# zhvng/open-musiclm

Measured on NVIDIA H100. Metric: coarse-stage training tokens/sec (positions fed to the transformer per optimiser step / step time), higher is better.
Workload: dtype bf16 (fp16 operands for the forward GEMMs on LayerNorm outputs x weights; fp32 accumulate)

## Files before the change

### open-musiclm_b200/csrc/attn_bwd_tc.cu

```cuda
#include "common.cuh"
#include "ptx.cuh"
#include "../../include/omlm_b200.h"
#include <stdlib.h>
#include <algorithm>
#include <array>
#include <functional>
#include <map>
#include <mutex>
#include <vector>

namespace omlm {

constexpr int kBtThreads = 384;
constexpr int kBtBQ = 64, kBtBK = 128;
constexpr float kBtL2e = 1.4426950408889634f;

constexpr int kBoK = 0, kBoV = 16384, kBoQ = 32768 , kBoDO = 49152 ;
constexpr int kBoP = 65536 , kBoDS = 81920 , kBoBar = 98304 ;
constexpr int kBoSds = 98368;
constexpr int kBtMaxSmem = 232448;
constexpr int kBtSdsLd = 72;
constexpr int kBoWin = kBoSds + 2 * 64 * kBtSdsLd * 4;

static int bt_win_ld(int h) { return ((62 + h) / h + 64 + 23) / 32 * 32 + 8; }

__device__ __forceinline__ float bt_ex2(float x) {
  float y;
  asm("ex2.approx.ftz.f32 %0, %1;" : "=f"(y) : "f"(x));
  return y;
}
__device__ __forceinline__ void bt_red2(float* addr, float a, float b) {
  asm volatile("red.global.add.v2.f32 [%0], {%1, %2};" ::"l"(addr), "f"(a), "f"(b) : "memory");
}
__device__ __forceinline__ void bt_cp_async4(float* dst, const float* src) {
  asm volatile("cp.async.ca.shared.global [%0], [%1], 4;" ::"r"(smem_u32(dst)), "l"(src) : "memory");
}

__device__ __forceinline__ int bt_ld_acquire(const int* p) {
  int v;
  asm volatile("ld.acquire.gpu.global.b32 %0, [%1];" : "=r"(v) : "l"(p) : "memory");
  return v;
}
__device__ __forceinline__ unsigned long long bt_globaltimer() {
  unsigned long long t;
  asm volatile("mov.u64 %0, %%globaltimer;" : "=l"(t));
  return t;
}
__device__ __noinline__ void bt_wait_turn(const int* ctr, int turn, int* err) {
  const unsigned long long t0 = bt_globaltimer();
  while (bt_ld_acquire(ctr) != turn) {
    if (*reinterpret_cast<volatile int*>(err) != 0) return;
    if (bt_globaltimer() - t0 > 4000000000ull) { atomicExch(err, 1); return; }
    __nanosleep(64);
  }
}
__device__ __forceinline__ void bt_pass_turn(int* ctr) {
  asm volatile("red.release.gpu.global.add.s32 [%0], 1;" ::"l"(ctr) : "memory");
}

struct BtDet {
  int* turn_dq;
  int* turn_kv;
  int* meta;
  int* err;
  float* dpart;
};

template <bool DET>
__global__ void __launch_bounds__(kBtThreads, 1)
attn_bwd_tc_kernel(const __grid_constant__ CUtensorMap tmQ, const __grid_constant__ CUtensorMap tmDO,
                   const __grid_constant__ CUtensorMap tmKV, const float* __restrict__ lse2, const float* __restrict__ dsum,
                   const float* __restrict__ table, int table_ld, const unsigned char* __restrict__ key_mask,
                   float* __restrict__ dqn, float* __restrict__ dkvn, float* __restrict__ dtable, int N, int h, float scale,
                   int Wacc, int win_ld, int tiles_per_chunk, int nbatch, const BtDet det) {
  extern __shared__ __align__(1024) uint8_t smem_raw[];
  uint8_t* smem = smem_raw + ((1024u - (smem_u32(smem_raw) & 1023u)) & 1023u);
  uint64_t* bars = reinterpret_cast<uint64_t*>(smem + kBoBar);
  uint64_t* kv_full = bars + 0;
  uint64_t* qd_full = bars + 1;
  uint64_t* qd_empty = bars + 3;
  float* dacc = reinterpret_cast<float*>(smem + kBoWin) + 2 * h * win_ld;

  const int wg = threadIdx.x >> 7, lane = threadIdx.x & 31;
  const int R = N * h;
  const int n_rt = (R + kBtBQ - 1) / kBtBQ;
  const int n_kt = (N + kBtBK - 1) / kBtBK;
  const int b = blockIdx.x % nbatch;
  int u = blockIdx.x / nbatch, kt = 0;
  for (; kt < n_kt; ++kt) {
    const int cnt = (n_rt - (kt * kBtBK * h) / kBtBQ + tiles_per_chunk - 1) / tiles_per_chunk;
    if (u < cnt) break;
    u -= cnt;
  }
  const int j0 = kt * kBtBK;
  const int rt0 = (j0 * h) / kBtBQ + u * tiles_per_chunk;
  const int rt1 = min(n_rt, rt0 + tiles_per_chunk);
  const int T = rt1 - rt0;
  const int i_lo = (rt0 * kBtBQ) / h, i_hi = min(N - 1, (rt1 * kBtBQ - 1) / h);
  const int dmin = max(0, i_lo - j0 - (kBtBK - 1));
  const int wacc_used = i_hi - j0 - dmin + 1;

  if (threadIdx.x == 0) {
    tma_prefetch_desc(&tmQ); tma_prefetch_desc(&tmDO); tma_prefetch_desc(&tmKV);
    mbar_init(kv_full, 1);
    for (int i = 0; i < 2; ++i) { mbar_init(&qd_full[i], 1); mbar_init(&qd_empty[i], 2); }
    fence_barrier_init();
  }
  for (int x = threadIdx.x; x < 2 * h * Wacc; x += blockDim.x) dacc[x] = 0.f;
  __syncthreads();

  if (wg == 0) {
    asm volatile("setmaxnreg.dec.sync.aligned.u32 40;");
    if (threadIdx.x == 0) {
      mbar_expect_tx(kv_full, 2 * 16384);
      tma_load_2d(smem + kBoK, &tmKV, kv_full, 0, b * N + j0);
      tma_load_2d(smem + kBoV, &tmKV, kv_full, 64, b * N + j0);
      for (int t = 0; t < T; ++t) {
        const int st = t & 1;
        mbar_wait(&qd_empty[st], ((t >> 1) & 1) ^ 1);
        mbar_expect_tx(&qd_full[st], 2 * 8192);
        tma_load_2d(smem + kBoQ + st * 8192, &tmQ, &qd_full[st], 0, b * R + (rt0 + t) * kBtBQ);
        tma_load_2d(smem + kBoDO + st * 8192, &tmDO, &qd_full[st], 0, b * R + (rt0 + t) * kBtBQ);
      }
    }
  } else {
    asm volatile("setmaxnreg.inc.sync.aligned.u32 232;");
    const int cw = wg - 1;
    const int wq = (threadIdx.x >> 5) & 3, qr = lane >> 2, qc = lane & 3;
    const bool leader = (threadIdx.x & 127) == 0;
    const int kbase = j0 + cw * 64;
    const uint32_t sk = smem_u32(smem + kBoK) + cw * 8192, sv = smem_u32(smem + kBoV) + cw * 8192;
    uint8_t* p_tile = smem + kBoP + cw * 8192;
    uint8_t* ds_tile = smem + kBoDS + cw * 8192;
    float* sdsf = reinterpret_cast<float*>(smem + kBoSds) + cw * 64 * kBtSdsLd;
    float* win = reinterpret_cast<float*>(smem + kBoWin) + cw * h * win_ld;
    float* wacc = dacc + cw * h * Wacc;
    const int tid128 = threadIdx.x & 127;
    const uint32_t sp = smem_u32(p_tile), sds = smem_u32(ds_tile);
    const float sc2 = scale * kBtL2e;
    uint32_t vis = 0;
#pragma unroll
    for (int c = 0; c < 8; ++c)
#pragma unroll
      for (int e = 0; e < 2; ++e) {
        const int j = kbase + 8 * c + 2 * qc + e;
        if (j < N && (key_mask == nullptr || key_mask[static_cast<long long>(b) * N + j] != 0)) vis |= 1u << (2 * c + e);
      }
    auto fetch_tile = [&](int rb, float (&lse)[2], float (&D)[2]) {
      const int it_lo = min(rb, R - 1) / h, it_hi = min(rb + kBtBQ - 1, R - 1) / h;
      const int win_w = it_hi - it_lo + 64, dlo = it_lo - kbase - 63;
      for (int hh = tid128 / win_w, w = tid128 - hh * win_w; hh < h;) {
        if (dlo + w >= 0) bt_cp_async4(win + hh * win_ld + w, table + hh * static_cast<long>(table_ld) + dlo + w);
        for (w += 128; w >= win_w; ++hh) w -= win_w;
      }
      asm volatile("cp.async.commit_group;" ::: "memory");
#pragma unroll
      for (int hr = 0; hr < 2; ++hr) {
        const int rc = min(rb + wq * 16 + qr + hr * 8, R - 1);
        lse[hr] = lse2[static_cast<long long>(b) * R + rc];
        D[hr] = dsum[static_cast<long long>(b) * R + rc];
      }
    };
    float lse_t[2], D_t[2];
    fetch_tile(rt0 * kBtBQ, lse_t, D_t);
    float dv[32], dk[32];
#pragma unroll
    for (int x = 0; x < 32; ++x) { dv[x] = 0.f; dk[x] = 0.f; }
    mbar_wait(kv_full, 0);
    for (int t = 0; t < T; ++t) {
      const int st = t & 1;
      const int rbase = (rt0 + t) * kBtBQ;
      const uint32_t sq = smem_u32(smem + kBoQ + st * 8192), sdo = smem_u32(smem + kBoDO + st * 8192);
      mbar_wait(&qd_full[st], (t >> 1) & 1);
      float s[32], dp[32];
      wgmma_fence();
#pragma unroll
      for (int ks = 0; ks < 4; ++ks) {
        Wgmma<64, false>::ss<0, 0>(s, make_smem_desc(sq + ks * 32, 16, 1024), make_smem_desc(sk + ks * 32, 16, 1024), ks > 0 ? 1u : 0u);
        Wgmma<64, false>::ss<0, 0>(dp, make_smem_desc(sdo + ks * 32, 16, 1024), make_smem_desc(sv + ks * 32, 16, 1024), ks > 0 ? 1u : 0u);
      }
      wgmma_commit();
      const int it_lo = min(rbase, R - 1) / h, it_hi = min(rbase + kBtBQ - 1, R - 1) / h;
      asm volatile("cp.async.wait_all;" ::: "memory");
      asm volatile("bar.sync %0, 128;" ::"r"(1 + cw) : "memory");
      wgmma_wait<0>();
      wgmma_reg_fence(s);
      wgmma_reg_fence(dp);
#pragma unroll
      for (int hr = 0; hr < 2; ++hr) {
        const int lr = wq * 16 + qr + hr * 8;
        const int r = rbase + lr;
        const bool row_ok = r < R;
        const int rc = min(r, R - 1);
        const int i = rc / h, hh = rc - i * h;
        const float lse = lse_t[hr], D = D_t[hr];
        const float* wrow = win + hh * win_ld + i - it_lo + 63 - 2 * qc;
        const int dcol = i - kbase - 2 * qc;
        uint8_t* prow = p_tile + lr * 128;
        uint8_t* drow = ds_tile + lr * 128;
        float wv[16];
#pragma unroll
        for (int x = 0; x < 16; ++x) wv[x] = wrow[-8 * (x >> 1) - (x & 1)];
#pragma unroll
        for (int c = 0; c < 8; ++c) {
          float pp[2], dd[2];
#pragma unroll
          for (int e = 0; e < 2; ++e) {
            const bool live = row_ok && ((vis >> (2 * c + e)) & 1u) && dcol >= 8 * c + e;
            const float x = s[4 * c + 2 * hr + e];
            pp[e] = live ? bt_ex2(fmaf(x, sc2, wv[2 * c + e] * kBtL2e) - lse) : 0.f;
            dd[e] = pp[e] * (dp[4 * c + 2 * hr + e] - D);
          }
          *reinterpret_cast<float2*>(sdsf + lr * kBtSdsLd + 8 * c + 2 * qc) = make_float2(dd[0], dd[1]);
          const uint32_t off = static_cast<uint32_t>(((c ^ (lr & 7)) << 4) + 4 * qc);
          *reinterpret_cast<uint32_t*>(prow + off) = pack_bf16x2(pp[0], pp[1]);
          *reinterpret_cast<uint32_t*>(drow + off) = pack_bf16x2(dd[0], dd[1]);
        }
      }
      fence_proxy_async();
      asm volatile("bar.sync %0, 128;" ::"r"(1 + cw) : "memory");
      if (t + 1 < T) fetch_tile(rbase + kBtBQ, lse_t, D_t);
      float dq[32];
      wgmma_fence();
#pragma unroll
      for (int ks = 0; ks < 4; ++ks) {
        Wgmma<64, false>::ss<1, 1>(dv, make_smem_desc(sp + ks * 2048, 8192, 1024), make_smem_desc(sdo + ks * 2048, 8192, 1024), 1u);
        Wgmma<64, false>::ss<1, 1>(dk, make_smem_desc(sds + ks * 2048, 8192, 1024), make_smem_desc(sq + ks * 2048, 8192, 1024), 1u);
        Wgmma<64, false>::ss<0, 1>(dq, make_smem_desc(sds + ks * 32, 16, 1024), make_smem_desc(sk + ks * 2048, 8192, 1024), ks > 0 ? 1u : 0u);
      }
      wgmma_commit();
      {
        const int dlo = max(0, it_lo - kbase - 63), dhi = it_hi - kbase;
        const int W = dhi - dlo + 1;
        const int q0 = rbase / h, r0 = rbase - q0 * h;
        const int q1 = (rbase + kBtBQ - 1) / h, r1 = rbase + kBtBQ - 1 - q1 * h;
        for (int hh = W > 0 ? tid128 / W : h, w = W > 0 ? tid128 - hh * W : 0; hh < h;) {
          const int dl = dlo + w;
          const int i0 = max(q0 + (hh < r0 ? 1 : 0), kbase + dl);
          const int i1 = min(min(q1 - (hh > r1 ? 1 : 0), N - 1), kbase + dl + 63);
          const float* src = sdsf + (i0 * h + hh - rbase) * kBtSdsLd + (i0 - dl - kbase);
          const int stride = h * kBtSdsLd + 1;
          float sum = 0.f;
          for (int i = i0; i <= i1; i += 8, src += 8 * stride) {
            float x[8];
#pragma unroll
            for (int k = 0; k < 8; ++k) x[k] = i + k <= i1 ? src[k * stride] : 0.f;
#pragma unroll
            for (int k = 0; k < 8; ++k)
              if (i + k <= i1) sum += x[k];
          }
          wacc[hh * Wacc + dl - dmin] += sum;
          for (w += 128; w >= W && hh < h; ++hh) w -= W;
        }
      }
      wgmma_wait<0>();
      wgmma_reg_fence(dq);
      wgmma_reg_fence(dv);
      wgmma_reg_fence(dk);
      asm volatile("bar.sync %0, 128;" ::"r"(1 + cw) : "memory");
      if (leader) mbar_arrive(&qd_empty[st]);
      int* turn = DET ? det.turn_dq + static_cast<long>(b) * n_rt + rt0 + t : nullptr;
      if constexpr (DET) {
        if (leader) bt_wait_turn(turn, 2 * kt + cw, det.err);
        asm volatile("bar.sync %0, 128;" ::"r"(1 + cw) : "memory");
      }
#pragma unroll
      for (int hr = 0; hr < 2; ++hr) {
        const int r = rbase + wq * 16 + qr + hr * 8;
        if (r < R) {
          float* dst = dqn + (static_cast<long long>(b) * R + r) * 64 + 2 * qc;
#pragma unroll
          for (int c = 0; c < 8; ++c) bt_red2(dst + 8 * c, dq[4 * c + 2 * hr] * scale, dq[4 * c + 2 * hr + 1] * scale);
        }
      }
      if constexpr (DET) {
        __threadfence();
        asm volatile("bar.sync %0, 128;" ::"r"(1 + cw) : "memory");
        if (leader) bt_pass_turn(turn);
      }
    }
    int* kv_turn = DET ? det.turn_kv + (static_cast<long>(b) * n_kt + kt) * 2 + cw : nullptr;
    if constexpr (DET) {
      if (leader) bt_wait_turn(kv_turn, u, det.err);
      asm volatile("bar.sync %0, 128;" ::"r"(1 + cw) : "memory");
    }
#pragma unroll
    for (int hr = 0; hr < 2; ++hr) {
      const int j = kbase + wq * 16 + qr + hr * 8;
      if (j < N) {
        float* dst = dkvn + (static_cast<long long>(b) * N + j) * 128 + 2 * qc;
#pragma unroll
        for (int c = 0; c < 8; ++c) {
          bt_red2(dst + 8 * c, dk[4 * c + 2 * hr] * scale, dk[4 * c + 2 * hr + 1] * scale);
          bt_red2(dst + 64 + 8 * c, dv[4 * c + 2 * hr], dv[4 * c + 2 * hr + 1]);
        }
      }
    }
    if constexpr (DET) {
      __threadfence();
      asm volatile("bar.sync %0, 128;" ::"r"(1 + cw) : "memory");
      if (leader) bt_pass_turn(kv_turn);
    }
    asm volatile("bar.sync 3, 256;" ::: "memory");
    if constexpr (DET) {
      float* up = det.dpart + static_cast<long>(blockIdx.x) * h * Wacc;
      for (int x = threadIdx.x - 128; x < h * wacc_used; x += 256) {
        const int hh = x / wacc_used, w = x - hh * wacc_used;
        up[hh * Wacc + w] = dacc[hh * Wacc + w] + dacc[(h + hh) * Wacc + w];
      }
      if (threadIdx.x == 128) { det.meta[2 * blockIdx.x] = dmin; det.meta[2 * blockIdx.x + 1] = wacc_used; }
    } else {
      for (int x = threadIdx.x - 128; x < h * wacc_used; x += 256) {
        const int hh = x / wacc_used, w = x - hh * wacc_used;
        const float v = dacc[hh * Wacc + w] + dacc[(h + hh) * Wacc + w];
        if (v != 0.f) atomicAdd(dtable + hh * static_cast<long>(table_ld) + dmin + w, v);
      }
    }
  }
}

__global__ void __launch_bounds__(256)
attn_bwd_dtable_reduce_kernel(const float* __restrict__ dpart, const int* __restrict__ meta, int units, int h, int Wacc,
                              float* __restrict__ dtable, int table_ld, int N) {
  const int x = blockIdx.x * blockDim.x + threadIdx.x;
  if (x >= h * N) return;
  const int hh = x / N, d = x - hh * N;
  float* dst = dtable + hh * static_cast<long>(table_ld) + d;
  float acc = *dst;
  for (int u = 0; u < units; ++u) {
    const int w = d - __ldg(meta + 2 * u);
    if (w >= 0 && w < __ldg(meta + 2 * u + 1)) acc += dpart[(static_cast<long>(u) * h + hh) * Wacc + w];
  }
  *dst = acc;
}

__global__ void __launch_bounds__(256)
attn_bwd_tc_dsum_kernel(const __nv_bfloat16* __restrict__ d_o, const __nv_bfloat16* __restrict__ o,
                        float* __restrict__ dsum, long rows, float* __restrict__ dqn, float* __restrict__ dkvn, long kv_vec4) {
  const long tid = static_cast<long>(blockIdx.x) * blockDim.x + threadIdx.x;
  const long r = tid >> 3;
  const int sub = threadIdx.x & 7;
  float s = 0.f;
  for (long i = tid; i < kv_vec4; i += static_cast<long>(gridDim.x) * blockDim.x)
    reinterpret_cast<float4*>(dkvn)[i] = make_float4(0.f, 0.f, 0.f, 0.f);
  if (r < rows) {
    float4* zq = reinterpret_cast<float4*>(dqn + r * 64 + sub * 8);
    zq[0] = make_float4(0.f, 0.f, 0.f, 0.f);
    zq[1] = make_float4(0.f, 0.f, 0.f, 0.f);
    const uint4 a = *reinterpret_cast<const uint4*>(d_o + r * 64 + sub * 8);
    const uint4 bq = *reinterpret_cast<const uint4*>(o + r * 64 + sub * 8);
    const uint32_t aa[4] = {a.x, a.y, a.z, a.w}, bb[4] = {bq.x, bq.y, bq.z, bq.w};
#pragma unroll
    for (int i = 0; i < 4; ++i) {
      const float2 x = unpack_bf16x2(aa[i]), y = unpack_bf16x2(bb[i]);
      s += x.x * y.x + x.y * y.y;
    }
  }
  s += __shfl_xor_sync(0xffffffffu, s, 1);
  s += __shfl_xor_sync(0xffffffffu, s, 2);
  s += __shfl_xor_sync(0xffffffffu, s, 4);
  if (r < rows && sub == 0) dsum[r] = s;
}

}

namespace omlm {

struct BtConfig {
  int tiles_per_chunk, wacc, win_ld, smem_bytes, units_per_batch, n_row_tiles, n_key_tiles;
};

template <class Fits>
static int bt_pick_chunk(int B, int n_row_tiles, int n_key_tiles, int heads, Fits fits) {
  static std::mutex mu;
  static std::map<std::array<int, 5>, int> memo;
  const int sms = num_sms();
  const std::array<int, 5> key{B, n_row_tiles, n_key_tiles, heads, sms};
  std::lock_guard<std::mutex> lock(mu);
  const auto hit = memo.find(key);
  if (hit != memo.end()) return hit->second;
  int best_T = 1;
  long best = -1;
  std::vector<long> busy(sms);
  for (int T = 1; T <= std::min(16, n_row_tiles); ++T) {
    if (!fits(T)) break;
    std::fill(busy.begin(), busy.end(), 0L);
    for (int kt = 0; kt < n_key_tiles; ++kt) {
      const int first = (kt * kBtBK * heads) / kBtBQ;
      for (int rt = first; rt < n_row_tiles; rt += T) {
        const long cost = std::min(T, n_row_tiles - rt) + 1;
        for (int b = 0; b < B; ++b) {
          std::pop_heap(busy.begin(), busy.end(), std::greater<long>());
          busy.back() += cost;
          std::push_heap(busy.begin(), busy.end(), std::greater<long>());
        }
      }
    }
    const long makespan = *std::max_element(busy.begin(), busy.end());
    if (best < 0 || makespan <= best) { best = makespan; best_T = T; }
  }
  memo[key] = best_T;
  return best_T;
}

static int bt_config(int B, int N, int heads, BtConfig* cfg) {
  const long R = static_cast<long>(N) * heads;
  const int n_row_tiles = static_cast<int>((R + kBtBQ - 1) / kBtBQ);
  const int n_key_tiles = (N + kBtBK - 1) / kBtBK;
  const int win_ld = bt_win_ld(heads);
  auto wacc_of = [&](int T) { return (T * kBtBQ + heads - 1) / heads + kBtBK + 2; };
  auto smem_of = [&](int T) { return kBoWin + 2 * heads * (win_ld + wacc_of(T)) * 4 + 1024; };
  auto units_of = [&](int T) {
    long units = 0;
    for (int kt = 0; kt < n_key_tiles; ++kt) {
      const int first = (kt * kBtBK * heads) / kBtBQ;
      units += (n_row_tiles - first + T - 1) / T;
    }
    return units;
  };
  OMLM_CHECK_ARG(smem_of(1) <= kBtMaxSmem, "attn_bwd_tc: too many heads (%d) for the shared-memory bias tables", heads);
  int tiles_per_chunk = bt_pick_chunk(B, n_row_tiles, n_key_tiles, heads, [&](int T) { return smem_of(T) <= kBtMaxSmem; });
  if (const char* e = getenv("OMLM_ATTN_BWD_T")) {
    const int T = atoi(e);
    if (T >= 1 && T <= n_row_tiles && smem_of(T) <= kBtMaxSmem) tiles_per_chunk = T;
  }
  cfg->tiles_per_chunk = tiles_per_chunk;
  cfg->wacc = wacc_of(tiles_per_chunk);
  cfg->win_ld = win_ld;
  cfg->smem_bytes = smem_of(tiles_per_chunk);
  cfg->units_per_batch = static_cast<int>(units_of(tiles_per_chunk));
  cfg->n_row_tiles = n_row_tiles;
  cfg->n_key_tiles = n_key_tiles;
  return 0;
}

static int bt_ints(int B, const BtConfig& c) {
  return B * c.n_row_tiles + 2 * B * c.n_key_tiles + 2 * B * c.units_per_batch + 1;
}

static int attn_bwd_tc_impl(const void* qn, const void* kvn, const void* d_o, const void* o, const float* lse2,
                            const float* table, int table_ld, const unsigned char* key_mask, float* dsum_scratch,
                            float* dqn, float* dkvn, float* dtable, int B, int N, int heads, float scale, bool det,
                            float* ws, long ws_bytes, int* iws, long iws_count, void* stream) {
  OMLM_CHECK_ARG(B > 0 && N > 0 && heads > 0, "attn_bwd_tc: bad shape");
  OMLM_CHECK_ARG(table_ld >= N, "attn_bwd_tc: bias table shorter than the sequence");
  auto st = reinterpret_cast<cudaStream_t>(stream);
  const long R = static_cast<long>(N) * heads;
  const long rows = static_cast<long>(B) * R;
  BtConfig cfg;
  int rc = bt_config(B, N, heads, &cfg);
  if (rc) return rc;
  const int units = B * cfg.units_per_batch;
  BtDet dp{nullptr, nullptr, nullptr, nullptr, nullptr};
  if (det) {
    OMLM_CHECK_ARG(ws != nullptr && iws != nullptr && ws_bytes >= static_cast<long>(units) * heads * cfg.wacc * 4 &&
                   iws_count >= bt_ints(B, cfg), "attn_bwd_tc_det: workspace too small (see omlm_attn_bwd_tc_det_workspace)");
    dp.turn_dq = iws;
    dp.turn_kv = iws + static_cast<long>(B) * cfg.n_row_tiles;
    dp.meta = dp.turn_kv + 2L * B * cfg.n_key_tiles;
    dp.err = iws + iws_count - 1;
    dp.dpart = ws;
    OMLM_CUDA(cudaMemsetAsync(iws, 0, (static_cast<long>(B) * cfg.n_row_tiles + 2L * B * cfg.n_key_tiles) * sizeof(int), st));
  }
  OMLM_KLAUNCH((attn_bwd_tc_dsum_kernel), static_cast<int>((rows * 8 + 255) / 256), 256, 0, st,
      reinterpret_cast<const __nv_bfloat16*>(d_o), reinterpret_cast<const __nv_bfloat16*>(o), dsum_scratch, rows,
      dqn, dkvn, static_cast<long>(B) * N * 128 / 4);
  OMLM_LAUNCH_CHECK();
  CUtensorMap tmQ, tmDO, tmKV;
  rc = make_tmap_bf16_2d(&tmQ, qn, 64, static_cast<uint64_t>(rows), 128, 64, kBtBQ);
  if (rc) return rc;
  rc = make_tmap_bf16_2d(&tmDO, d_o, 64, static_cast<uint64_t>(rows), 128, 64, kBtBQ);
  if (rc) return rc;
  rc = make_tmap_bf16_2d(&tmKV, kvn, 128, static_cast<uint64_t>(B) * N, 256, 64, kBtBK);
  if (rc) return rc;
  auto kern = det ? attn_bwd_tc_kernel<true> : attn_bwd_tc_kernel<false>;
  static int configured[2] = {0, 0};
  if (configured[det] < cfg.smem_bytes) {
    OMLM_CUDA(cudaFuncSetAttribute(kern, cudaFuncAttributeMaxDynamicSharedMemorySize, cfg.smem_bytes));
    configured[det] = cfg.smem_bytes;
  }
  OMLM_KLAUNCH((kern), units, kBtThreads, cfg.smem_bytes, st,
      tmQ, tmDO, tmKV, lse2, dsum_scratch, table, table_ld, key_mask, dqn, dkvn, dtable, N, heads, scale,
      cfg.wacc, cfg.win_ld, cfg.tiles_per_chunk, B, dp);
  OMLM_LAUNCH_CHECK();
  if (det) {
    OMLM_KLAUNCH((attn_bwd_dtable_reduce_kernel), (heads * N + 255) / 256, 256, 0, st,
        static_cast<const float*>(dp.dpart), static_cast<const int*>(dp.meta), units, heads, cfg.wacc, dtable, table_ld, N);
    OMLM_LAUNCH_CHECK();
  }
  return 0;
}

}

extern "C" int omlm_attn_bwd_tc(const void* qn, const void* kvn, const void* d_o, const void* o, const float* lse2,
                                const float* table, int table_ld, const unsigned char* key_mask, float* dsum_scratch,
                                float* dqn, float* dkvn, float* dtable, int B, int N, int heads,
                                float scale, void* stream) {
  return omlm::attn_bwd_tc_impl(qn, kvn, d_o, o, lse2, table, table_ld, key_mask, dsum_scratch, dqn, dkvn, dtable, B, N, heads,
                                scale, false, nullptr, 0, nullptr, 0, stream);
}

extern "C" int omlm_attn_bwd_tc_det(const void* qn, const void* kvn, const void* d_o, const void* o, const float* lse2,
                                    const float* table, int table_ld, const unsigned char* key_mask, float* dsum_scratch,
                                    float* dqn, float* dkvn, float* dtable, int B, int N, int heads, float scale,
                                    float* ws, long ws_bytes, int* iws, long iws_count, void* stream) {
  return omlm::attn_bwd_tc_impl(qn, kvn, d_o, o, lse2, table, table_ld, key_mask, dsum_scratch, dqn, dkvn, dtable, B, N, heads,
                                scale, true, ws, ws_bytes, iws, iws_count, stream);
}

extern "C" int omlm_attn_bwd_tc_det_workspace(int B, int N, int heads, long* ws_bytes, long* iws_count) {
  using namespace omlm;
  OMLM_CHECK_ARG(B > 0 && N > 0 && heads > 0 && ws_bytes != nullptr && iws_count != nullptr, "attn_bwd_tc_det_workspace: bad arguments");
  BtConfig cfg;
  const int rc = bt_config(B, N, heads, &cfg);
  if (rc) return rc;
  *ws_bytes = static_cast<long>(B) * cfg.units_per_batch * heads * cfg.wacc * 4;
  *iws_count = bt_ints(B, cfg);
  return 0;
}
```

### open-musiclm_b200/csrc/common.cuh

```cuda
#pragma once
#include <cuda_runtime.h>
#include <cuda_bf16.h>
#include <cuda_fp16.h>
#include <cuda.h>
#include <stdint.h>
#include <stdio.h>

namespace omlm {

void set_last_error(const char* fmt, ...);
#define OMLM_CHECK_ARG(cond, ...)          \
  do {                                     \
    if (!(cond)) {                         \
      ::omlm::set_last_error(__VA_ARGS__); \
      return 1;                            \
    }                                      \
  } while (0)
#define OMLM_CUDA(expr)                                                                       \
  do {                                                                                        \
    cudaError_t _e = (expr);                                                                  \
    if (_e != cudaSuccess) {                                                                  \
      ::omlm::set_last_error("%s:%d %s -> %s", __FILE__, __LINE__, #expr, cudaGetErrorString(_e)); \
      return 1000 + static_cast<int>(_e);                                                     \
    }                                                                                         \
  } while (0)
#define OMLM_LAUNCH_CHECK() OMLM_CUDA(cudaGetLastError())

int make_tmap_bf16_2d(CUtensorMap* out, const void* gptr, uint64_t dim0, uint64_t dim1,
                      uint64_t pitch_bytes, uint32_t box0, uint32_t box1);

int make_tmap_2d(CUtensorMap* out, int elem_bytes, const void* gptr, uint64_t dim0, uint64_t dim1, uint64_t pitch_bytes,
                 uint32_t box0, uint32_t box1);

int make_tmap_bf16_3d(CUtensorMap* out, const void* gptr, uint64_t dim0, uint64_t dim1, uint64_t dim2,
                      uint64_t pitch1_bytes, uint64_t pitch2_bytes, uint32_t box0, uint32_t box1);

int num_sms();

template <typename... KArgs, typename... Args>
inline cudaError_t launch_k(void (*kern)(KArgs...), dim3 grid, dim3 block, size_t smem, cudaStream_t stream, Args&&... args) {
  cudaLaunchConfig_t cfg = {};
  cfg.gridDim = grid; cfg.blockDim = block; cfg.dynamicSmemBytes = smem; cfg.stream = stream;
  return cudaLaunchKernelEx(&cfg, kern, static_cast<KArgs>(args)...);
}
#define OMLM_KLAUNCH(kern, grid, block, smem, stream, ...)                                                   \
  do {                                                                                                       \
    cudaError_t _le = ::omlm::launch_k(kern, dim3(grid), dim3(block), smem, stream, __VA_ARGS__);            \
    if (_le != cudaSuccess) {                                                                                \
      ::omlm::set_last_error("%s:%d launch of %s -> %s", __FILE__, __LINE__, #kern, cudaGetErrorString(_le)); \
      return 1000 + static_cast<int>(_le);                                                                   \
    }                                                                                                        \
  } while (0)

__device__ __forceinline__ float warp_sum(float v) {
#pragma unroll
  for (int o = 16; o > 0; o >>= 1) v += __shfl_xor_sync(0xffffffffu, v, o);
  return v;
}
__device__ __forceinline__ float warp_max(float v) {
#pragma unroll
  for (int o = 16; o > 0; o >>= 1) v = fmaxf(v, __shfl_xor_sync(0xffffffffu, v, o));
  return v;
}
__device__ __forceinline__ uint32_t pack_bf16x2(float lo, float hi) {
  __nv_bfloat162 t = __floats2bfloat162_rn(lo, hi);
  return *reinterpret_cast<uint32_t*>(&t);
}
__device__ __forceinline__ float2 unpack_bf16x2(uint32_t v) {
  __nv_bfloat162 t = *reinterpret_cast<__nv_bfloat162*>(&v);
  return __bfloat1622float2(t);
}
__device__ __forceinline__ float bf16_round(float x) {
  return __bfloat162float(__float2bfloat16_rn(x));
}
enum : int { kFmtBF16 = 0, kFmtF32 = 1, kFmtF16 = 2 };
__device__ __forceinline__ uint32_t pack_f16x2(float lo, float hi) {
  uint32_t r;
  asm("cvt.rn.satfinite.f16x2.f32 %0, %1, %2;" : "=r"(r) : "f"(hi), "f"(lo));
  return r;
}
__device__ __forceinline__ float2 unpack_f16x2(uint32_t v) {
  __half2 t = *reinterpret_cast<__half2*>(&v);
  return __half22float2(t);
}
template <bool F16>
__device__ __forceinline__ uint32_t pack16x2(float lo, float hi) {
  if constexpr (F16) return pack_f16x2(lo, hi); else return pack_bf16x2(lo, hi);
}
template <bool F16>
__device__ __forceinline__ float2 unpack16x2(uint32_t v) {
  if constexpr (F16) return unpack_f16x2(v); else return unpack_bf16x2(v);
}

__device__ __forceinline__ float2 fma2(float2 a, float2 b, float2 c) { return make_float2(fmaf(a.x, b.x, c.x), fmaf(a.y, b.y, c.y)); }
__device__ __forceinline__ float2 mul2(float2 a, float2 b) { return make_float2(__fmul_rn(a.x, b.x), __fmul_rn(a.y, b.y)); }
__device__ __forceinline__ float2 add2(float2 a, float2 b) { return make_float2(__fadd_rn(a.x, b.x), __fadd_rn(a.y, b.y)); }
__device__ __forceinline__ float2 splat2(float v) { return make_float2(v, v); }
__device__ __forceinline__ float rcp_approx(float x) {
  float r;
  asm("rcp.approx.ftz.f32 %0, %1;" : "=f"(r) : "f"(x));
  return r;
}
__device__ __forceinline__ float ex2_approx(float x) {
  float r;
  asm("ex2.approx.ftz.f32 %0, %1;" : "=f"(r) : "f"(x));
  return r;
}

__device__ __forceinline__ void normal_cdf_pdf(float x, float& cdf, float& pdf) {
  const float e = ex2_approx(-0.72134752044448170f * x * x);
  const float t = rcp_approx(fmaf(0.23164189f, fabsf(x), 1.f));
  float p = fmaf(0.5f * 1.061405429f, t, 0.5f * -1.453152027f);
  p = fmaf(p, t, 0.5f * 1.421413741f);
  p = fmaf(p, t, 0.5f * -0.284496736f);
  p = fmaf(p, t, 0.5f * 0.254829592f);
  const float half_erfc = p * t * e;
  cdf = x >= 0.f ? 1.f - half_erfc : half_erfc;
  pdf = 0.3989422804014327f * e;
}
__device__ __forceinline__ void normal_cdf_pdf2(float2 x, float2& cdf, float2& pdf) {
  const float2 q = mul2(mul2(x, x), splat2(-0.72134752044448170f));
  const float2 e = make_float2(ex2_approx(q.x), ex2_approx(q.y));
  const float2 t = make_float2(rcp_approx(fmaf(0.23164189f, fabsf(x.x), 1.f)), rcp_approx(fmaf(0.23164189f, fabsf(x.y), 1.f)));
  float2 p = fma2(splat2(0.5f * 1.061405429f), t, splat2(0.5f * -1.453152027f));
  p = fma2(p, t, splat2(0.5f * 1.421413741f));
  p = fma2(p, t, splat2(0.5f * -0.284496736f));
  p = fma2(p, t, splat2(0.5f * 0.254829592f));
  const float2 h = mul2(mul2(p, t), e);
  cdf = make_float2(x.x >= 0.f ? 1.f - h.x : h.x, x.y >= 0.f ? 1.f - h.y : h.y);
  pdf = mul2(e, splat2(0.3989422804014327f));
}
__device__ __forceinline__ float gelu_erf(float x) {
  float c, p;
  normal_cdf_pdf(x, c, p);
  return x * c;
}
__device__ __forceinline__ float2 gelu_erf2(float2 x) {
  float2 c, p;
  normal_cdf_pdf2(x, c, p);
  return mul2(x, c);
}

__device__ __forceinline__ uint4 philox4x32(uint32_t c0, uint32_t c1, uint32_t c2, uint32_t c3,
                                            uint32_t k0, uint32_t k1) {
#pragma unroll
  for (int i = 0; i < 7; ++i) {
    const uint32_t hi0 = __umulhi(0xD2511F53u, c0), lo0 = 0xD2511F53u * c0;
    const uint32_t hi1 = __umulhi(0xCD9E8D57u, c2), lo1 = 0xCD9E8D57u * c2;
    const uint32_t n0 = hi1 ^ c1 ^ k0, n1 = lo1, n2 = hi0 ^ c3 ^ k1, n3 = lo0;
    c0 = n0; c1 = n1; c2 = n2; c3 = n3;
    k0 += 0x9E3779B9u; k1 += 0xBB67AE85u;
  }
  return make_uint4(c0, c1, c2, c3);
}

}
```

### open-musiclm_b200/csrc/host.cu

```cuda
#include "common.cuh"
#include "../../include/omlm_b200.h"
#include <cudaTypedefs.h>
#include <stdarg.h>
#include <string.h>
#include <mutex>

namespace omlm {

static thread_local char g_err[1024] = "";

void set_last_error(const char* fmt, ...) {
  va_list ap;
  va_start(ap, fmt);
  vsnprintf(g_err, sizeof(g_err), fmt, ap);
  va_end(ap);
}

static PFN_cuTensorMapEncodeTiled_v12000 g_encode = nullptr;
static std::once_flag g_encode_once;

static void resolve_encode() {
  void* fn = nullptr;
  cudaDriverEntryPointQueryResult qres;
  cudaError_t e = cudaGetDriverEntryPoint("cuTensorMapEncodeTiled", &fn, cudaEnableDefault, &qres);
  if (e == cudaSuccess && qres == cudaDriverEntryPointSuccess) {
    g_encode = reinterpret_cast<PFN_cuTensorMapEncodeTiled_v12000>(fn);
  }
}

int make_tmap_bf16_2d(CUtensorMap* out, const void* gptr, uint64_t dim0, uint64_t dim1,
                      uint64_t pitch_bytes, uint32_t box0, uint32_t box1) {
  std::call_once(g_encode_once, resolve_encode);
  OMLM_CHECK_ARG(g_encode != nullptr, "cuTensorMapEncodeTiled not available (no CUDA driver?)");
  OMLM_CHECK_ARG((reinterpret_cast<uintptr_t>(gptr) & 15) == 0, "TMA base pointer must be 16B aligned");
  OMLM_CHECK_ARG((pitch_bytes & 15) == 0, "TMA row pitch must be a multiple of 16B (got %llu)",
                 (unsigned long long)pitch_bytes);
  OMLM_CHECK_ARG(box0 * 2 == 128 && box1 >= 1 && box1 <= 256, "bad TMA box %u x %u", box0, box1);
  cuuint64_t dims[2] = {dim0, dim1};
  cuuint64_t strides[1] = {pitch_bytes};
  cuuint32_t box[2] = {box0, box1};
  cuuint32_t estr[2] = {1, 1};
  CUresult r = g_encode(out, CU_TENSOR_MAP_DATA_TYPE_BFLOAT16, 2, const_cast<void*>(gptr), dims,
                        strides, box, estr, CU_TENSOR_MAP_INTERLEAVE_NONE,
                        CU_TENSOR_MAP_SWIZZLE_128B, CU_TENSOR_MAP_L2_PROMOTION_L2_256B,
                        CU_TENSOR_MAP_FLOAT_OOB_FILL_NONE);
  OMLM_CHECK_ARG(r == CUDA_SUCCESS, "cuTensorMapEncodeTiled failed with CUresult %d", (int)r);
  return 0;
}

int make_tmap_2d(CUtensorMap* out, int elem_bytes, const void* gptr, uint64_t dim0, uint64_t dim1, uint64_t pitch_bytes,
                 uint32_t box0, uint32_t box1) {
  std::call_once(g_encode_once, resolve_encode);
  OMLM_CHECK_ARG(g_encode != nullptr, "cuTensorMapEncodeTiled not available (no CUDA driver?)");
  OMLM_CHECK_ARG(elem_bytes == 2 || elem_bytes == 4, "make_tmap_2d: element size %d", elem_bytes);
  OMLM_CHECK_ARG((reinterpret_cast<uintptr_t>(gptr) & 15) == 0 && (pitch_bytes & 15) == 0, "TMA base / pitch must be 16B aligned");
  OMLM_CHECK_ARG(box0 * elem_bytes == 128 && box1 >= 1 && box1 <= 256, "bad TMA box %u x %u", box0, box1);
  cuuint64_t dims[2] = {dim0, dim1};
  cuuint64_t strides[1] = {pitch_bytes};
  cuuint32_t box[2] = {box0, box1};
  cuuint32_t estr[2] = {1, 1};
  CUresult r = g_encode(out, elem_bytes == 4 ? CU_TENSOR_MAP_DATA_TYPE_FLOAT32 : CU_TENSOR_MAP_DATA_TYPE_BFLOAT16, 2,
                        const_cast<void*>(gptr), dims, strides, box, estr, CU_TENSOR_MAP_INTERLEAVE_NONE,
                        CU_TENSOR_MAP_SWIZZLE_128B, CU_TENSOR_MAP_L2_PROMOTION_L2_256B, CU_TENSOR_MAP_FLOAT_OOB_FILL_NONE);
  OMLM_CHECK_ARG(r == CUDA_SUCCESS, "cuTensorMapEncodeTiled failed with CUresult %d", (int)r);
  return 0;
}

int make_tmap_bf16_3d(CUtensorMap* out, const void* gptr, uint64_t dim0, uint64_t dim1, uint64_t dim2,
                      uint64_t pitch1_bytes, uint64_t pitch2_bytes, uint32_t box0, uint32_t box1) {
  std::call_once(g_encode_once, resolve_encode);
  OMLM_CHECK_ARG(g_encode != nullptr, "cuTensorMapEncodeTiled not available (no CUDA driver?)");
  OMLM_CHECK_ARG((reinterpret_cast<uintptr_t>(gptr) & 15) == 0 && (pitch1_bytes & 15) == 0 && (pitch2_bytes & 15) == 0,
                 "TMA 3-D map: base and pitches must be 16B aligned");
  OMLM_CHECK_ARG(box0 * 2 == 128 && box1 >= 1 && box1 <= 256, "bad TMA box %u x %u", box0, box1);
  cuuint64_t dims[3] = {dim0, dim1, dim2};
  cuuint64_t strides[2] = {pitch1_bytes, pitch2_bytes};
  cuuint32_t box[3] = {box0, box1, 1};
  cuuint32_t estr[3] = {1, 1, 1};
  CUresult r = g_encode(out, CU_TENSOR_MAP_DATA_TYPE_BFLOAT16, 3, const_cast<void*>(gptr), dims, strides, box, estr,
                        CU_TENSOR_MAP_INTERLEAVE_NONE, CU_TENSOR_MAP_SWIZZLE_128B, CU_TENSOR_MAP_L2_PROMOTION_L2_256B,
                        CU_TENSOR_MAP_FLOAT_OOB_FILL_NONE);
  OMLM_CHECK_ARG(r == CUDA_SUCCESS, "cuTensorMapEncodeTiled (3-D) failed with CUresult %d", (int)r);
  return 0;
}

int num_sms() {
  static int n = 0;
  if (n == 0) {
    int dev = 0;
    cudaGetDevice(&dev);
    cudaDeviceGetAttribute(&n, cudaDevAttrMultiProcessorCount, dev);
  }
  return n;
}

}

extern "C" {

const char* omlm_last_error(void) { return omlm::g_err; }

int omlm_abi_version(void) { return OMLM_B200_ABI_VERSION; }

int omlm_num_sms(void) { return omlm::num_sms(); }

int omlm_device_check(void) {
  int dev = 0;
  OMLM_CUDA(cudaGetDevice(&dev));
  int major = 0, minor = 0;
  OMLM_CUDA(cudaDeviceGetAttribute(&major, cudaDevAttrComputeCapabilityMajor, dev));
  OMLM_CUDA(cudaDeviceGetAttribute(&minor, cudaDevAttrComputeCapabilityMinor, dev));
  OMLM_CHECK_ARG(major == 9 && minor == 0, "libomlm_b200 is built for sm_90a only; device is sm_%d%d", major, minor);
  return 0;
}

}
```

Baseline: 747,000.

## Offload bias-window loads to producer warps and use TMA reduce-add for dQ

```diff
diff --git a/open-musiclm_b200/csrc/attn_bwd_tc.cu b/open-musiclm_b200/csrc/attn_bwd_tc.cu
--- a/open-musiclm_b200/csrc/attn_bwd_tc.cu
+++ b/open-musiclm_b200/csrc/attn_bwd_tc.cu
@@ -16,11 +16,12 @@
 constexpr float kBtL2e = 1.4426950408889634f;
 
 constexpr int kBoK = 0, kBoV = 16384, kBoQ = 32768 , kBoDO = 49152 ;
-constexpr int kBoP = 65536 , kBoDS = 81920 , kBoBar = 98304 ;
-constexpr int kBoSds = 98368;
+constexpr int kBoP = 65536 , kBoDS = 81920 ;
+constexpr int kBoSds = 98304;
 constexpr int kBtMaxSmem = 232448;
 constexpr int kBtSdsLd = 72;
-constexpr int kBoWin = kBoSds + 2 * 64 * kBtSdsLd * 4;
+constexpr int kBoBar = kBoSds + 2 * 64 * kBtSdsLd * 4;
+constexpr int kBoWin = kBoBar + 80;
 
 static int bt_win_ld(int h) { return ((62 + h) / h + 64 + 23) / 32 * 32 + 8; }
 
@@ -34,6 +35,14 @@
 }
 __device__ __forceinline__ void bt_cp_async4(float* dst, const float* src) {
   asm volatile("cp.async.ca.shared.global [%0], [%1], 4;" ::"r"(smem_u32(dst)), "l"(src) : "memory");
+}
+__device__ __forceinline__ void bt_cp_async_arrive(uint64_t* bar) {
+  asm volatile("cp.async.mbarrier.arrive.noinc.shared::cta.b64 [%0];" ::"r"(smem_u32(bar)) : "memory");
+}
+__device__ __forceinline__ void bt_tma_reduce_add_3d(const CUtensorMap* m, const void* smem_src, int c0, int c1, int c2) {
+  asm volatile("cp.reduce.async.bulk.tensor.3d.global.shared::cta.add.tile.bulk_group [%0, {%2, %3, %4}], [%1];"
+               ::"l"(reinterpret_cast<uint64_t>(m)), "r"(smem_u32(smem_src)), "r"(c0), "r"(c1), "r"(c2)
+               : "memory");
 }
 
 __device__ __forceinline__ int bt_ld_acquire(const int* p) {
@@ -69,9 +78,10 @@
 template <bool DET>
 __global__ void __launch_bounds__(kBtThreads, 1)
 attn_bwd_tc_kernel(const __grid_constant__ CUtensorMap tmQ, const __grid_constant__ CUtensorMap tmDO,
-                   const __grid_constant__ CUtensorMap tmKV, const float* __restrict__ lse2, const float* __restrict__ dsum,
+                   const __grid_constant__ CUtensorMap tmKV, const __grid_constant__ CUtensorMap tmDQ,
+                   const float* __restrict__ lse2, const float* __restrict__ dsum,
                    const float* __restrict__ table, int table_ld, const unsigned char* __restrict__ key_mask,
-                   float* __restrict__ dqn, float* __restrict__ dkvn, float* __restrict__ dtable, int N, int h, float scale,
+                   float* __restrict__ dkvn, float* __restrict__ dtable, int N, int h, float scale,
                    int Wacc, int win_ld, int tiles_per_chunk, int nbatch, const BtDet det) {
   extern __shared__ __align__(1024) uint8_t smem_raw[];
   uint8_t* smem = smem_raw + ((1024u - (smem_u32(smem_raw) & 1023u)) & 1023u);
@@ -79,6 +89,8 @@
   uint64_t* kv_full = bars + 0;
   uint64_t* qd_full = bars + 1;
   uint64_t* qd_empty = bars + 3;
+  uint64_t* win_full = bars + 5;
+  uint64_t* win_empty = bars + 7;
   float* dacc = reinterpret_cast<float*>(smem + kBoWin) + 2 * h * win_ld;
 
   const int wg = threadIdx.x >> 7, lane = threadIdx.x & 31;
@@ -101,9 +113,12 @@
   const int wacc_used = i_hi - j0 - dmin + 1;
 
   if (threadIdx.x == 0) {
-    tma_prefetch_desc(&tmQ); tma_prefetch_desc(&tmDO); tma_prefetch_desc(&tmKV);
+    tma_prefetch_desc(&tmQ); tma_prefetch_desc(&tmDO); tma_prefetch_desc(&tmKV); tma_prefetch_desc(&tmDQ);
     mbar_init(kv_full, 1);
-    for (int i = 0; i < 2; ++i) { mbar_init(&qd_full[i], 1); mbar_init(&qd_empty[i], 2); }
+    for (int i = 0; i < 2; ++i) {
+      mbar_init(&qd_full[i], 1); mbar_init(&qd_empty[i], 2);
+      mbar_init(&win_full[i], 32); mbar_init(&win_empty[i], 1);
+    }
     fence_barrier_init();
   }
   for (int x = threadIdx.x; x < 2 * h * Wacc; x += blockDim.x) dacc[x] = 0.f;
@@ -111,7 +126,24 @@
 
   if (wg == 0) {
     asm volatile("setmaxnreg.dec.sync.aligned.u32 40;");
-    if (threadIdx.x == 0) {
+    const int warp = threadIdx.x >> 5;
+    if (warp == 1 || warp == 2) {
+      const int cw = warp - 1;
+      const int kbase = j0 + cw * 64;
+      float* win = reinterpret_cast<float*>(smem + kBoWin) + cw * h * win_ld;
+      for (int t = 0; t < T; ++t) {
+        if (t > 0) mbar_wait(&win_empty[cw], (t - 1) & 1);
+        const int rb = (rt0 + t) * kBtBQ;
+        const int it_lo = min(rb, R - 1) / h, it_hi = min(rb + kBtBQ - 1, R - 1) / h;
+        const int win_w = it_hi - it_lo + 64, dlo = it_lo - kbase - 63;
+        for (int hh = 0, w = lane; hh < h;) {
+          if (dlo + w >= 0) bt_cp_async4(win + hh * win_ld + w, table + hh * static_cast<long>(table_ld) + dlo + w);
+          w += 32;
+          if (w >= win_w) { w -= win_w; ++hh; }
+        }
+        bt_cp_async_arrive(&win_full[cw]);
+      }
+    } else if (threadIdx.x == 0) {
       mbar_expect_tx(kv_full, 2 * 16384);
       tma_load_2d(smem + kBoK, &tmKV, kv_full, 0, b * N + j0);
       tma_load_2d(smem + kBoV, &tmKV, kv_full, 64, b * N + j0);
@@ -146,14 +178,7 @@
         const int j = kbase + 8 * c + 2 * qc + e;
         if (j < N && (key_mask == nullptr || key_mask[static_cast<long long>(b) * N + j] != 0)) vis |= 1u << (2 * c + e);
       }
-    auto fetch_tile = [&](int rb, float (&lse)[2], float (&D)[2]) {
-      const int it_lo = min(rb, R - 1) / h, it_hi = min(rb + kBtBQ - 1, R - 1) / h;
-      const int win_w = it_hi - it_lo + 64, dlo = it_lo - kbase - 63;
-      for (int hh = tid128 / win_w, w = tid128 - hh * win_w; hh < h;) {
-        if (dlo + w >= 0) bt_cp_async4(win + hh * win_ld + w, table + hh * static_cast<long>(table_ld) + dlo + w);
-        for (w += 128; w >= win_w; ++hh) w -= win_w;
-      }
-      asm volatile("cp.async.commit_group;" ::: "memory");
+    auto fetch_rows = [&](int rb, float (&lse)[2], float (&D)[2]) {
 #pragma unroll
       for (int hr = 0; hr < 2; ++hr) {
         const int rc = min(rb + wq * 16 + qr + hr * 8, R - 1);
@@ -162,7 +187,7 @@
       }
     };
     float lse_t[2], D_t[2];
-    fetch_tile(rt0 * kBtBQ, lse_t, D_t);
+    fetch_rows(rt0 * kBtBQ, lse_t, D_t);
     float dv[32], dk[32];
 #pragma unroll
     for (int x = 0; x < 32; ++x) { dv[x] = 0.f; dk[x] = 0.f; }
@@ -181,7 +206,8 @@
       }
       wgmma_commit();
       const int it_lo = min(rbase, R - 1) / h, it_hi = min(rbase + kBtBQ - 1, R - 1) / h;
-      asm volatile("cp.async.wait_all;" ::: "memory");
+      if (leader) tma_store_wait_read<0>();
+      mbar_wait(&win_full[cw], t & 1);
       asm volatile("bar.sync %0, 128;" ::"r"(1 + cw) : "memory");
       wgmma_wait<0>();
       wgmma_reg_fence(s);
@@ -219,7 +245,8 @@
       }
       fence_proxy_async();
       asm volatile("bar.sync %0, 128;" ::"r"(1 + cw) : "memory");
-      if (t + 1 < T) fetch_tile(rbase + kBtBQ, lse_t, D_t);
+      if (leader && t + 1 < T) mbar_arrive(&win_empty[cw]);
+      if (t + 1 < T) fetch_rows(rbase + kBtBQ, lse_t, D_t);
       float dq[32];
       wgmma_fence();
 #pragma unroll
@@ -259,26 +286,33 @@
       wgmma_reg_fence(dk);
       asm volatile("bar.sync %0, 128;" ::"r"(1 + cw) : "memory");
       if (leader) mbar_arrive(&qd_empty[st]);
-      int* turn = DET ? det.turn_dq + static_cast<long>(b) * n_rt + rt0 + t : nullptr;
-      if constexpr (DET) {
-        if (leader) bt_wait_turn(turn, 2 * kt + cw, det.err);
-        asm volatile("bar.sync %0, 128;" ::"r"(1 + cw) : "memory");
-      }
 #pragma unroll
       for (int hr = 0; hr < 2; ++hr) {
-        const int r = rbase + wq * 16 + qr + hr * 8;
-        if (r < R) {
-          float* dst = dqn + (static_cast<long long>(b) * R + r) * 64 + 2 * qc;
-#pragma unroll
-          for (int c = 0; c < 8; ++c) bt_red2(dst + 8 * c, dq[4 * c + 2 * hr] * scale, dq[4 * c + 2 * hr + 1] * scale);
-        }
-      }
-      if constexpr (DET) {
-        __threadfence();
-        asm volatile("bar.sync %0, 128;" ::"r"(1 + cw) : "memory");
-        if (leader) bt_pass_turn(turn);
-      }
-    }
+        const int lr = wq * 16 + qr + hr * 8;
+#pragma unroll
+        for (int c = 0; c < 8; ++c) {
+          const int chunk = (2 * (c & 3) + (qc >> 1)) ^ (lr & 7);
+          *reinterpret_cast<float2*>(sdsf + (c >> 2) * 2048 + lr * 32 + chunk * 4 + 2 * (qc & 1)) =
+              make_float2(dq[4 * c + 2 * hr] * scale, dq[4 * c + 2 * hr + 1] * scale);
+        }
+      }
+      fence_proxy_async();
+      asm volatile("bar.sync %0, 128;" ::"r"(1 + cw) : "memory");
+      if (leader) {
+        int* turn = DET ? det.turn_dq + static_cast<long>(b) * n_rt + rt0 + t : nullptr;
+        if constexpr (DET) bt_wait_turn(turn, 2 * kt + cw, det.err);
+        bt_tma_reduce_add_3d(&tmDQ, sdsf, 0, rbase, b);
+        bt_tma_reduce_add_3d(&tmDQ, sdsf + 2048, 32, rbase, b);
+        tma_store_commit();
+        if constexpr (DET) {
+          tma_store_wait_all();
+          asm volatile("fence.proxy.async.global;" ::: "memory");
+          __threadfence();
+          bt_pass_turn(turn);
+        }
+      }
+    }
+    if (leader) tma_store_wait_read<0>();
     int* kv_turn = DET ? det.turn_kv + (static_cast<long>(b) * n_kt + kt) * 2 + cw : nullptr;
     if constexpr (DET) {
       if (leader) bt_wait_turn(kv_turn, u, det.err);
@@ -371,18 +405,18 @@
 };
 
 template <class Fits>
-static int bt_pick_chunk(int B, int n_row_tiles, int n_key_tiles, int heads, Fits fits) {
+static int bt_pick_chunk(int B, int n_row_tiles, int n_key_tiles, int heads, int max_T, Fits fits) {
   static std::mutex mu;
-  static std::map<std::array<int, 5>, int> memo;
+  static std::map<std::array<int, 6>, int> memo;
   const int sms = num_sms();
-  const std::array<int, 5> key{B, n_row_tiles, n_key_tiles, heads, sms};
+  const std::array<int, 6> key{B, n_row_tiles, n_key_tiles, heads, max_T, sms};
   std::lock_guard<std::mutex> lock(mu);
   const auto hit = memo.find(key);
   if (hit != memo.end()) return hit->second;
   int best_T = 1;
   long best = -1;
   std::vector<long> busy(sms);
-  for (int T = 1; T <= std::min(16, n_row_tiles); ++T) {
+  for (int T = 1; T <= std::min(max_T, n_row_tiles); ++T) {
     if (!fits(T)) break;
     std::fill(busy.begin(), busy.end(), 0L);
     for (int kt = 0; kt < n_key_tiles; ++kt) {
@@ -403,7 +437,7 @@
   return best_T;
 }
 
-static int bt_config(int B, int N, int heads, BtConfig* cfg) {
+static int bt_config(int B, int N, int heads, bool det, BtConfig* cfg) {
   const long R = static_cast<long>(N) * heads;
   const int n_row_tiles = static_cast<int>((R + kBtBQ - 1) / kBtBQ);
   const int n_key_tiles = (N + kBtBK - 1) / kBtBK;
@@ -419,7 +453,8 @@
     return units;
   };
   OMLM_CHECK_ARG(smem_of(1) <= kBtMaxSmem, "attn_bwd_tc: too many heads (%d) for the shared-memory bias tables", heads);
-  int tiles_per_chunk = bt_pick_chunk(B, n_row_tiles, n_key_tiles, heads, [&](int T) { return smem_of(T) <= kBtMaxSmem; });
+  int tiles_per_chunk = bt_pick_chunk(B, n_row_tiles, n_key_tiles, heads, det ? 16 : 24,
+                                      [&](int T) { return smem_of(T) <= kBtMaxSmem; });
   if (const char* e = getenv("OMLM_ATTN_BWD_T")) {
     const int T = atoi(e);
     if (T >= 1 && T <= n_row_tiles && smem_of(T) <= kBtMaxSmem) tiles_per_chunk = T;
@@ -448,7 +483,7 @@
   const long R = static_cast<long>(N) * heads;
   const long rows = static_cast<long>(B) * R;
   BtConfig cfg;
-  int rc = bt_config(B, N, heads, &cfg);
+  int rc = bt_config(B, N, heads, det, &cfg);
   if (rc) return rc;
   const int units = B * cfg.units_per_batch;
   BtDet dp{nullptr, nullptr, nullptr, nullptr, nullptr};
@@ -473,6 +508,10 @@
   if (rc) return rc;
   rc = make_tmap_bf16_2d(&tmKV, kvn, 128, static_cast<uint64_t>(B) * N, 256, 64, kBtBK);
   if (rc) return rc;
+  CUtensorMap tmDQ;
+  rc = make_tmap_3d(&tmDQ, 4, dqn, 64, static_cast<uint64_t>(R), static_cast<uint64_t>(B), 256, static_cast<uint64_t>(R) * 256,
+                    32, kBtBQ);
+  if (rc) return rc;
   auto kern = det ? attn_bwd_tc_kernel<true> : attn_bwd_tc_kernel<false>;
   static int configured[2] = {0, 0};
   if (configured[det] < cfg.smem_bytes) {
@@ -480,7 +519,7 @@
     configured[det] = cfg.smem_bytes;
   }
   OMLM_KLAUNCH((kern), units, kBtThreads, cfg.smem_bytes, st,
-      tmQ, tmDO, tmKV, lse2, dsum_scratch, table, table_ld, key_mask, dqn, dkvn, dtable, N, heads, scale,
+      tmQ, tmDO, tmKV, tmDQ, lse2, dsum_scratch, table, table_ld, key_mask, dkvn, dtable, N, heads, scale,
       cfg.wacc, cfg.win_ld, cfg.tiles_per_chunk, B, dp);
   OMLM_LAUNCH_CHECK();
   if (det) {
@@ -513,7 +552,7 @@
   using namespace omlm;
   OMLM_CHECK_ARG(B > 0 && N > 0 && heads > 0 && ws_bytes != nullptr && iws_count != nullptr, "attn_bwd_tc_det_workspace: bad arguments");
   BtConfig cfg;
-  const int rc = bt_config(B, N, heads, &cfg);
+  const int rc = bt_config(B, N, heads, true, &cfg);
   if (rc) return rc;
   *ws_bytes = static_cast<long>(B) * cfg.units_per_batch * heads * cfg.wacc * 4;
   *iws_count = bt_ints(B, cfg);
diff --git a/open-musiclm_b200/csrc/common.cuh b/open-musiclm_b200/csrc/common.cuh
--- a/open-musiclm_b200/csrc/common.cuh
+++ b/open-musiclm_b200/csrc/common.cuh
@@ -32,8 +32,8 @@
 int make_tmap_2d(CUtensorMap* out, int elem_bytes, const void* gptr, uint64_t dim0, uint64_t dim1, uint64_t pitch_bytes,
                  uint32_t box0, uint32_t box1);
 
-int make_tmap_bf16_3d(CUtensorMap* out, const void* gptr, uint64_t dim0, uint64_t dim1, uint64_t dim2,
-                      uint64_t pitch1_bytes, uint64_t pitch2_bytes, uint32_t box0, uint32_t box1);
+int make_tmap_3d(CUtensorMap* out, int elem_bytes, const void* gptr, uint64_t dim0, uint64_t dim1, uint64_t dim2,
+                 uint64_t pitch1_bytes, uint64_t pitch2_bytes, uint32_t box0, uint32_t box1);
 
 int num_sms();
 
diff --git a/open-musiclm_b200/csrc/host.cu b/open-musiclm_b200/csrc/host.cu
--- a/open-musiclm_b200/csrc/host.cu
+++ b/open-musiclm_b200/csrc/host.cu
@@ -66,18 +66,20 @@
   return 0;
 }
 
-int make_tmap_bf16_3d(CUtensorMap* out, const void* gptr, uint64_t dim0, uint64_t dim1, uint64_t dim2,
-                      uint64_t pitch1_bytes, uint64_t pitch2_bytes, uint32_t box0, uint32_t box1) {
+int make_tmap_3d(CUtensorMap* out, int elem_bytes, const void* gptr, uint64_t dim0, uint64_t dim1, uint64_t dim2,
+                 uint64_t pitch1_bytes, uint64_t pitch2_bytes, uint32_t box0, uint32_t box1) {
   std::call_once(g_encode_once, resolve_encode);
   OMLM_CHECK_ARG(g_encode != nullptr, "cuTensorMapEncodeTiled not available (no CUDA driver?)");
+  OMLM_CHECK_ARG(elem_bytes == 2 || elem_bytes == 4, "make_tmap_3d: element size %d", elem_bytes);
   OMLM_CHECK_ARG((reinterpret_cast<uintptr_t>(gptr) & 15) == 0 && (pitch1_bytes & 15) == 0 && (pitch2_bytes & 15) == 0,
                  "TMA 3-D map: base and pitches must be 16B aligned");
-  OMLM_CHECK_ARG(box0 * 2 == 128 && box1 >= 1 && box1 <= 256, "bad TMA box %u x %u", box0, box1);
+  OMLM_CHECK_ARG(box0 * elem_bytes == 128 && box1 >= 1 && box1 <= 256, "bad TMA box %u x %u", box0, box1);
   cuuint64_t dims[3] = {dim0, dim1, dim2};
   cuuint64_t strides[2] = {pitch1_bytes, pitch2_bytes};
   cuuint32_t box[3] = {box0, box1, 1};
   cuuint32_t estr[3] = {1, 1, 1};
-  CUresult r = g_encode(out, CU_TENSOR_MAP_DATA_TYPE_BFLOAT16, 3, const_cast<void*>(gptr), dims, strides, box, estr,
+  CUresult r = g_encode(out, elem_bytes == 4 ? CU_TENSOR_MAP_DATA_TYPE_FLOAT32 : CU_TENSOR_MAP_DATA_TYPE_BFLOAT16, 3,
+                        const_cast<void*>(gptr), dims, strides, box, estr,
                         CU_TENSOR_MAP_INTERLEAVE_NONE, CU_TENSOR_MAP_SWIZZLE_128B, CU_TENSOR_MAP_L2_PROMOTION_L2_256B,
                         CU_TENSOR_MAP_FLOAT_OOB_FILL_NONE);
   OMLM_CHECK_ARG(r == CUDA_SUCCESS, "cuTensorMapEncodeTiled (3-D) failed with CUresult %d", (int)r);
```

Result: faster. 760,800 (median of 6 runs) (+1.9%).
